# maxjiang93/space_time_pde

Hardware: AMD Instinct MI355X
Metric: query-points/sec (fwd+PDE-residual bwd), rb2d 128^3 latent (higher is better)
Workload: dtype f32; 1 GPU; BASELINE configs[1]: latent [1,32,128,128,32], 2^20 query points, RB2 (3 transport + continuity), ImNet nf=32 softplus, L1 losses, backward to ImNet + UNet3d parameters; points=1048576, parallelism=points sharded x1, unet=UNet3d(igres=(32, 128, 128), nf=16, mf=256) fwd+bwd inside the timed step

## Files before the change

### include/stpde_hip.h

```cpp
#ifndef STPDE_HIP_H
#define STPDE_HIP_H

#ifdef __cplusplus
extern "C" {
#endif

#define STPDE_OK 0
#define STPDE_E_BADARG 1
#define STPDE_E_UNSUPPORTED 2
#define STPDE_E_LAUNCH 3

#define STPDE_ACT_TANH 0
#define STPDE_ACT_RELU 1
#define STPDE_ACT_SOFTPLUS 2
#define STPDE_ACT_ELU 3
#define STPDE_ACT_SWISH 4
#define STPDE_ACT_LEAKYRELU 5

#define STPDE_XT 3
#define STPDE_PBAR_SLOTS 64

typedef struct {
  int S1;
  int S2;
  int pair0[6];
  int pair1[6];
  int act;
  float act_param;
  int combo;
  float alpha[6];
} stpde_jet_cfg;

int stpde_version(void);
int stpde_last_error(char* buf, unsigned long n);
#define STPDE_TUNE_CONV3_LDS_OFF 0
#define STPDE_TUNE_CONV3_LDS_MINBLK 1
#define STPDE_TUNE_CONV3_LDS_GX 2
#define STPDE_TUNE_CONV_WGRAD_LDS_GX 3
#define STPDE_TUNE_CONV1_WGRAD_LDS_GX 4
#define STPDE_TUNE_WGRAD_FP32_SWAP 5
#define STPDE_TUNE_FC2_BWD_FUSED 6
#define STPDE_TUNE_COUNT 7
int stpde_tune(const char* name, int value);
int stpde_trace_enable(int on);
long stpde_trace_read(char* buf, unsigned long n);

typedef struct {
  int P, N, B, n0, n1, n2, C;
  int p_base;
  float lo_c[3], hi_c[3], cube[3];
  float alpha[6];
} stpde_gather_desc;
int stpde_lig_gather(const stpde_gather_desc* d, const float* pts, const float* latent, float* X, float* XR,
                     float* coef, int* cell, float* cw , void* stream);

typedef struct {
  int ntiles, KT, MT, first_hidden;
  stpde_jet_cfg cfg;
  int mfma_bf16;
  int packed;
  int det;
} stpde_layer_desc;
int stpde_jet_layer_fwd(const stpde_layer_desc* d, const float* in_pre, const float* X, const float* Wh_pack,
                        const float* Ws_pack, const float* tanc, const float* W0s_pack, const float* tanc0,
                        float* out_pre, const float* cw ,
                        const void* Wh_pack_bf16, float* z0, void* stream);

int stpde_jet_tail_fwd(const stpde_jet_cfg* cfg, int ntiles, int nf16, const float* in_pre2, const float* X,
                       const float* const* Wh_pack, const float* const* Ws_pack, const float* const* tanc,
                       float* const* out_pre, const float* cw, void* stream);

int stpde_jet_tail_fwd_p(const stpde_jet_cfg* cfg, int ntiles, int nf16, const float* in_pre2, const float* X,
                         const float* const* Wh_pack, const float* const* Ws_pack, const float* const* tanc,
                         float* const* out_pre, const float* cw, int packed, const void* const* Wh16_pack, void* stream);

int stpde_jet_tail_bwd(const stpde_jet_cfg* cfg, int ntiles, int nf16, const float* abar5, const float* const* WhT_pack,
                       const float* const* pre, float* const* abar_out, const float* cw, float* act_param_bar,
                       void* stream);

int stpde_jet_tail_bwd_p(const stpde_jet_cfg* cfg, int ntiles, int nf16, const float* abar5, const float* const* WhT_pack,
                         const float* const* pre, float* const* abar_out, const float* cw, float* act_param_bar, int packed,
                         const void* const* WhT16_pack, void* stream);

int stpde_jet_layer_bwd(const stpde_layer_desc* d, const float* abar_out, const float* WhT_pack, float* in_pre,
                        const float* X, const float* W0s_pack, const float* tanc0, float* abar0, const float* cw,
                        float* act_param_bar, const void* WhT_pack_bf16 ,
                        float* abar0_tan, const float* z0, void* stream);

int stpde_jet_layer_bwd_to(const stpde_layer_desc* d, const float* abar_out, const float* WhT_pack, const float* in_pre,
                           float* abar_in, const float* cw, float* act_param_bar, const void* WhT_pack_bf16, void* stream);

int stpde_jet_wgrad(const stpde_layer_desc* d, int SP, const float* abar_out, const float* in_pre, const float* X,
                    const float* tanc0, float* dW_aug, const float* cw, void* stream);

int stpde_jet_fc1_bwd_supported(const stpde_layer_desc* d);
int stpde_jet_fc1_bwd(const stpde_layer_desc* d, const float* abar1, const void* WhT_pack_bf16, const float* z0,
                      const float* tanc0, const float* cw, const float* X, float* abar0, float* abar0_tan, float* dW_aug,
                      float* act_param_bar, void* stream);

int stpde_jet_fc2_bwd_supported(const stpde_layer_desc* d);
int stpde_jet_fc2_bwd(const stpde_layer_desc* d, const float* abar2, const float* WhT_pack, const float* pre1, const float* X,
                      const float* cw, float* abar1, float* dW_aug, float* act_param_bar, void* stream);

int stpde_lig_reduce_fwd(const stpde_jet_cfg* cfg, int S_mlp, int P, int n_out, const float* out_pre,
                         const float* coef, float* jets, long ldp, void* stream);
int stpde_lig_reduce_bwd(const stpde_jet_cfg* cfg, int S_mlp, int P, int n_out, const float* jets_bar, long ldp,
                         const float* coef, float* abar_out, void* stream);

int stpde_jet_tan0_reduce(int ntiles, int MT, const float* abar0_tan, float* dW_aug, int ldw, int det ,
                          void* stream);

typedef struct {
  int ntiles, nlayers, C, n1, n2;
  int MT[8];
  int SP[8];
  int packed[8];
  int S[8];
} stpde_xbar_desc;
int stpde_lig_xbar_scatter(const stpde_xbar_desc* d, const float* const* abar, const float* const* WsL_pack,
                           const int* cell, float* dlatent, void* stream);
int stpde_lig_xbar_rows(const stpde_xbar_desc* d, const float* const* abar, const float* const* WsL_pack,
                        float* xrows, void* stream);
int stpde_lig_dlatent_reduce(int B, int n0, int n1, int n2, int C, const float* xrows, const int* perm,
                             const int* start, float* dlatent, void* stream);

// ... 56 lines not shown
                        void* stream);

typedef struct {
  int P, N, B, dim, C;
  int n[4];
  float lo_c[4], hi_c[4], cube[4];
} stpde_interp_desc;
int stpde_interp_fwd(const stpde_interp_desc* d, const float* grid, const float* pts, float* out ,
                     float* corner_values , float* weights ,
                     float* x_relative , void* stream);
int stpde_interp_bwd_grid(const stpde_interp_desc* d, const float* pts, const float* out_bar,
                          const float* corner_bar, float* dgrid, void* stream);

typedef struct {
  int D, P, N, B, C;
  int p_base;
  int ntiles;
  int n[4];
  float lo_c[4], hi_c[4], cube[4];
} stpde_gather_nd_desc;
int stpde_lig_gather_nd(const stpde_gather_nd_desc* d, const float* pts, const float* latent, float* X,
                        float* cw , void* stream);
int stpde_lig_reduce_nd_fwd(int D, int P, int ntiles, int n_out, const float* out_pre ,
                            const float* cw, float* y, long ldp, void* stream);

int stpde_lig_reduce_nd_bwd(int D, int P, int ntiles, int n_out, const float* y_bar, long ldp, const float* cw,
                            float* abar_out , void* stream);
int stpde_lig_cell_nd(const stpde_gather_nd_desc* d, const float* pts, int* cell , void* stream);
int stpde_lig_dlatent_reduce_nd(int D, int B, const int* n , int C, const float* xrows, const int* perm,
                                const int* start, float* dlatent, void* stream);

int stpde_lig_coef_nd(const stpde_gather_nd_desc* d, const float* pts, float* coef , void* stream);
int stpde_lig_reduce_nd_jet_fwd(const stpde_jet_cfg* cfg, int S_mlp, int D, int P, int ntiles, int n_out,
                                const float* out_pre , const float* coef,
                                float* jets , long ldp, void* stream);

int stpde_lig_reduce_nd_jet_bwd(const stpde_jet_cfg* cfg, int S_mlp, int D, int P, int ntiles, int n_out,
                                const float* jets_bar , long ldp, const float* coef,
                                float* abar_out , void* stream);
int stpde_jet_wgrad_nd(const stpde_layer_desc* d, int SP, const float* abar_out, const float* in_pre, const float* X,
                       const float* tanc0, float* dW_aug, const float* cw, int ncoord, void* stream);
int stpde_jet_tan0_reduce_nd(int ntiles, int MT, const float* abar0_tan, float* dW_aug, int ldw, int det, int ncoord, void* stream);

typedef struct {
  int B, T, Z, X, Ci, Co, ksize;
  int det;
  int mfma_bf16;
} stpde_conv3d_desc;
#define STPDE_DET_K 6
int stpde_det_finalize(const void* acc, long n, float* out, void* stream);
int stpde_conv3d_fwd(const stpde_conv3d_desc* d, const float* x, const float* w_pack, const float* bias, float* y,
                     void* stream);
int stpde_conv3d_wgrad(const stpde_conv3d_desc* d, const float* x, const float* ybar, float* dW, void* stream);
int stpde_conv3d_wgrad_bias(const stpde_conv3d_desc* d, const float* x, const float* ybar, float* dW, float* dbias,
                            void* stream);

typedef struct {
  stpde_conv3d_desc d;
  const float* x;
  const float* w_pack;
  const float* bias;
  float* y;
  const float* x2;
  const float* w2_pack;
  float* y2;
  const float* wo2_pack;
  const float* bias2;
  const double* in_sums;
  const float* in_gamma;
  const float* in_beta;
  float* in_running_mean;
  float* in_running_var;
  float* in_stat;
  double* out_sums;
  const float* m;
  const float* m_stat;
  const float* m_gamma;
  const float* m_beta;
  float* m_bsum;
  int Ci2, Co2;
  float in_eps, in_momentum;
} stpde_conv3d_fused_args;
int stpde_conv3d_fused(const stpde_conv3d_fused_args* a, int* epilogue_done, void* stream);
int stpde_conv3d_wgrad_onload(const stpde_conv3d_desc* d, const float* x, const float* ybar, float* dW, float* dbias,
                              const float* in_stat, const float* in_gamma, const float* in_beta, void* stream);

#define STPDE_BN_REP 16
typedef struct {
  long N;
  int C, training, relu;
  float eps, momentum;
  int scratch_zeroed;
  int stats_mode;
  int reduce_done;
  int det;
} stpde_bn_desc;
int stpde_bn_fwd(const stpde_bn_desc* d, const float* x, const float* residual, const float* gamma, const float* beta,
                 float* running_mean, float* running_var, float* sums, float* stat, float* y, void* stream);
int stpde_bn_bwd(const stpde_bn_desc* d, const float* x, const float* y, const float* dy, const float* gamma,
                 const float* stat, float* bsum, float* dx, float* dresidual, float* dgamma, float* dbeta, void* stream);

typedef struct {
  int B, T, Z, X, C, ft, fz, fx;
} stpde_resample_desc;
int stpde_resample3d(const stpde_resample_desc* d, int mode, const float* in, const float* aux, float* out,
                     void* stream);

#define STPDE_RES_MAX_INS 192
enum {
  STPDE_RES_JET = 0, STPDE_RES_X, STPDE_RES_CONST, STPDE_RES_ADD, STPDE_RES_SUB, STPDE_RES_MUL, STPDE_RES_DIV,
  STPDE_RES_NEG, STPDE_RES_POWI, STPDE_RES_SIN, STPDE_RES_COS, STPDE_RES_EXP, STPDE_RES_LOG, STPDE_RES_SQRT,
  STPDE_RES_TANH, STPDE_RES_ABS, STPDE_RES_OUT,
  STPDE_RES_TAN, STPDE_RES_SINH, STPDE_RES_COSH, STPDE_RES_ASIN, STPDE_RES_ACOS, STPDE_RES_ATAN, STPDE_RES_ATAN2,
  STPDE_RES_POWC, STPDE_RES_POW, STPDE_RES_MIN, STPDE_RES_MAX, STPDE_RES_SIGN, STPDE_RES_STEP,
  STPDE_RES_LT, STPDE_RES_LE, STPDE_RES_EQ, STPDE_RES_NE, STPDE_RES_AND, STPDE_RES_OR, STPDE_RES_NOT,
  STPDE_RES_SEL, STPDE_RES_STEPC
};
#define STPDE_RES_SEL_THEN(b) ((int)((unsigned)(b) & 0xffffu))
#define STPDE_RES_SEL_ELSE(b) ((int)((unsigned)(b) >> 16))
typedef struct {
  int op, a, b;
  float c;
} stpde_res_ins;
int stpde_residual_fwd(const stpde_res_ins* prog_dev, int nins, int n_eq, int n_out, int P, const float* jets,
                       long ld_stream, long ld_channel, const float* x , float* res, void* stream);
int stpde_residual_bwd(const stpde_res_ins* prog_dev, int nins, int n_eq, int n_out, int P, const float* jets,
                       long ld_stream, long ld_channel, const float* x, const float* res_bar, float* jets_bar,
                       void* stream);
#define STPDE_RES_MAX_COEF 8
typedef struct {
  int n;
  int n_per_batch;
  int det;
  int per_batch[STPDE_RES_MAX_COEF];
  const float* value[STPDE_RES_MAX_COEF];
  float* bar[STPDE_RES_MAX_COEF];
} stpde_res_coefs;
int stpde_residual_coef_fwd(const stpde_res_ins* prog_dev, int nins, int n_eq, int n_out, int P, const float* jets,
                            long ld_stream, long ld_channel, const float* x, float* res, const stpde_res_coefs* coefs,
                            void* stream);
int stpde_residual_coef_bwd(const stpde_res_ins* prog_dev, int nins, int n_eq, int n_out, int P, const float* jets,
                            long ld_stream, long ld_channel, const float* x, const float* res_bar, float* jets_bar,
                            const stpde_res_coefs* coefs, void* stream);

#define STPDE_LOSS_L1 0
#define STPDE_LOSS_L2 1
#define STPDE_LOSS_HUBER 2
#define STPDE_LOSS_DET 16
int stpde_loss_sum(int kind, long n, const float* a, const float* b, float* out_sum, void* stream);
int stpde_loss_grad(int kind, long n, const float* a, const float* b, const float* grad_sum_dev, float* grad_a,
                    void* stream);

typedef struct {
  long n;
  float clip, beta1, beta2, eps, weight_decay, step_size, bias2_sqrt;
} stpde_adam_desc;
int stpde_clip_adam(const stpde_adam_desc* d, float* param, const float* grad, float* exp_avg, float* exp_avg_sq,
                    void* stream);
typedef struct {
  float* p;
  const float* g;
  float* m;
  float* v;
  long n;
  float step_size, bias2_sqrt;
} stpde_adam_tensor;
// ... 96 lines not shown
```

### space_time_pde_amd/_lib.py

```python
import ctypes as C
import os
import subprocess
import threading

_HERE = os.path.dirname(os.path.abspath(__file__))
_CSRC = os.path.join(_HERE, "csrc")
LIB_PATH = os.environ.get("STPDE_LIB") or os.path.join(_HERE, "libstpde_hip.so")
_SOURCES = ["jet_layer.hip", "jet_layer_s00.hip", "jet_layer_s03.hip", "jet_layer_s30.hip", "jet_layer_s31.hip", "jet_layer_s32.hip", "jet_layer_s34.hip", "jet_layer_s36.hip", "jet_tail.hip", "jet_wgrad.hip", "jet_wgrad_s00.hip", "jet_wgrad_s30.hip", "jet_wgrad_s31.hip", "jet_wgrad_s32.hip", "jet_wgrad_s34.hip", "jet_wgrad_s36.hip", "jet_fc1_bwd.hip", "jet_fc2_bwd.hip", "lig_gather_reduce.hip", "lig_pipeline.hip", "interp_nd.hip", "conv3d.hip", "conv3d_fused.hip", "optim.hip", "residual.hip", "bn.hip", "resample.hip", "sampler.hip", "sampler_median.hip", "api.cpp"]
_HIPFLAGS = ["--offload-arch=gfx950", "-O3", "-std=c++17", "-fPIC", "-ffp-contract=off", "-munsafe-fp-atomics",
             "--offload-compress"]

ABI_VERSION = 316

ACT_CODES = {"tanh": 0, "relu": 1, "softplus": 2, "elu": 3, "swish": 4, "leakyrelu": 5}
PBAR_SLOTS = 64
XT = 3


class JetCfg(C.Structure):
    _fields_ = [("S1", C.c_int), ("S2", C.c_int), ("pair0", C.c_int * 6), ("pair1", C.c_int * 6),
                ("act", C.c_int), ("act_param", C.c_float), ("combo", C.c_int), ("alpha", C.c_float * 6)]


class GatherDesc(C.Structure):
# ... 175 lines not shown
        objs.append(o)
        ostamp = o + ".srchash"
        owant = _source_hash([s] + _includes(s))
        if not force and os.path.exists(o) and os.path.exists(ostamp) and open(ostamp).read().strip() == owant:
            continue
        flags = _HIPFLAGS if s.endswith(".hip") else ["-O3", "-std=c++17", "-fPIC"]
        cmd = ["hipcc"] + flags + ["-c", s, "-o", o]
        if verbose:
            print(" ".join(cmd))
        procs.append((cmd, ostamp, owant, subprocess.Popen(cmd, stdout=subprocess.PIPE, stderr=subprocess.STDOUT)))
    for cmd, ostamp, owant, p in procs:
        out, _ = p.communicate()
        if p.returncode != 0:
            raise RuntimeError("hipcc failed: %s\n%s" % (" ".join(cmd), out.decode()))
        with open(ostamp, "w") as f:
            f.write(owant)
    cmd = ["hipcc", "--offload-arch=gfx950", "--offload-compress", "-shared", "-fPIC", "-o", LIB_PATH] + objs
    r = subprocess.run(cmd, stdout=subprocess.PIPE, stderr=subprocess.STDOUT)
    if r.returncode != 0:
        raise RuntimeError("link failed: %s\n%s" % (" ".join(cmd), r.stdout.decode()))
    with open(stamp, "w") as f:
        f.write(want)
    return LIB_PATH


_lib = None
_lock = threading.Lock()
_VP = C.c_void_p

_SIGNATURES = {
    "stpde_version": ([], C.c_int),
    "stpde_last_error": ([C.c_char_p, C.c_ulong], C.c_int),
    "stpde_tune": ([C.c_char_p, C.c_int], C.c_int),
    "stpde_trace_enable": ([C.c_int], C.c_int),
    "stpde_trace_read": ([C.c_char_p, C.c_ulong], C.c_long),
    "stpde_lig_gather": ([C.POINTER(GatherDesc), _VP, _VP, _VP, _VP, _VP, _VP, _VP, _VP], C.c_int),
    "stpde_lig_gather_nd": ([C.POINTER(GatherNdDesc), _VP, _VP, _VP, _VP, _VP], C.c_int),
    "stpde_lig_reduce_nd_fwd": ([C.c_int, C.c_int, C.c_int, C.c_int, _VP, _VP, _VP, C.c_long, _VP], C.c_int),
    "stpde_lig_reduce_nd_bwd": ([C.c_int, C.c_int, C.c_int, C.c_int, _VP, C.c_long, _VP, _VP, _VP], C.c_int),
    "stpde_lig_cell_nd": ([C.POINTER(GatherNdDesc), _VP, _VP, _VP], C.c_int),
    "stpde_lig_dlatent_reduce_nd": ([C.c_int, C.c_int, C.POINTER(C.c_int), C.c_int, _VP, _VP, _VP, _VP, _VP], C.c_int),
    "stpde_lig_coef_nd": ([C.POINTER(GatherNdDesc), _VP, _VP, _VP], C.c_int),
    "stpde_lig_reduce_nd_jet_fwd": ([C.POINTER(JetCfg), C.c_int, C.c_int, C.c_int, C.c_int, C.c_int, _VP, _VP, _VP, C.c_long,
                                     _VP], C.c_int),
    "stpde_lig_reduce_nd_jet_bwd": ([C.POINTER(JetCfg), C.c_int, C.c_int, C.c_int, C.c_int, C.c_int, _VP, C.c_long, _VP, _VP,
                                     _VP], C.c_int),
    "stpde_jet_wgrad_nd": ([C.POINTER(LayerDesc), C.c_int] + [_VP] * 6 + [C.c_int, _VP], C.c_int),
    "stpde_jet_tan0_reduce_nd": ([C.c_int, C.c_int, _VP, _VP, C.c_int, C.c_int, C.c_int, _VP], C.c_int),
    "stpde_jet_layer_fwd": ([C.POINTER(LayerDesc)] + [_VP] * 12, C.c_int),
    "stpde_jet_layer_bwd": ([C.POINTER(LayerDesc)] + [_VP] * 13, C.c_int),
    "stpde_jet_layer_bwd_to": ([C.POINTER(LayerDesc)] + [_VP] * 8, C.c_int),
    "stpde_jet_tail_fwd": ([C.POINTER(JetCfg), C.c_int, C.c_int, _VP, _VP, C.POINTER(_VP), C.POINTER(_VP), C.POINTER(_VP),
                            C.POINTER(_VP), _VP, _VP], C.c_int),
    "stpde_jet_tail_bwd": ([C.POINTER(JetCfg), C.c_int, C.c_int, _VP, C.POINTER(_VP), C.POINTER(_VP), C.POINTER(_VP), _VP,
                            _VP, _VP], C.c_int),
    "stpde_jet_tail_fwd_p": ([C.POINTER(JetCfg), C.c_int, C.c_int, _VP, _VP, C.POINTER(_VP), C.POINTER(_VP), C.POINTER(_VP),
                              C.POINTER(_VP), _VP, C.c_int, C.POINTER(_VP), _VP], C.c_int),
    "stpde_jet_tail_bwd_p": ([C.POINTER(JetCfg), C.c_int, C.c_int, _VP, C.POINTER(_VP), C.POINTER(_VP), C.POINTER(_VP), _VP,
                              _VP, C.c_int, C.POINTER(_VP), _VP], C.c_int),
    "stpde_jet_tan0_reduce": ([C.c_int, C.c_int, _VP, _VP, C.c_int, C.c_int, _VP], C.c_int),
    "stpde_jet_wgrad": ([C.POINTER(LayerDesc), C.c_int] + [_VP] * 7, C.c_int),
    "stpde_jet_fc1_bwd_supported": ([C.POINTER(LayerDesc)], C.c_int),
    "stpde_jet_fc1_bwd": ([C.POINTER(LayerDesc)] + [_VP] * 11, C.c_int),
    "stpde_jet_fc2_bwd_supported": ([C.POINTER(LayerDesc)], C.c_int),
    "stpde_jet_fc2_bwd": ([C.POINTER(LayerDesc)] + [_VP] * 9, C.c_int),
    "stpde_lig_reduce_fwd": ([C.POINTER(JetCfg), C.c_int, C.c_int, C.c_int, _VP, _VP, _VP, C.c_long, _VP], C.c_int),
    "stpde_lig_reduce_bwd": ([C.POINTER(JetCfg), C.c_int, C.c_int, C.c_int, _VP, C.c_long, _VP, _VP, _VP], C.c_int),
    "stpde_lig_xbar_scatter": ([C.POINTER(XbarDesc), C.POINTER(_VP), C.POINTER(_VP), _VP, _VP, _VP], C.c_int),
    "stpde_lig_xbar_rows": ([C.POINTER(XbarDesc), C.POINTER(_VP), C.POINTER(_VP), _VP, _VP], C.c_int),
    "stpde_lig_dlatent_reduce": ([C.c_int] * 5 + [_VP] * 5, C.c_int),
    "stpde_lig_imnet_jet_fwd": ([C.POINTER(ImNetPlanDesc), C.POINTER(JetCfg), C.POINTER(JetCfg), C.POINTER(GatherDesc), _VP,
                                 _VP, C.POINTER(LigWorkspace), _VP, C.c_long, C.c_int, _VP], C.c_int),
    "stpde_lig_imnet_jet_bwd": ([C.POINTER(ImNetPlanDesc), C.POINTER(JetCfg), C.POINTER(JetCfg), C.POINTER(JetCfg),
                                 C.POINTER(GatherDesc), C.POINTER(LigWorkspace), _VP, C.c_long, _VP, _VP, _VP, C.c_int, _VP],
                                C.c_int),
    "stpde_lig_sort_tmp_bytes": ([C.c_int, C.c_long], C.c_ulong),
    "stpde_lig_cell_sort": ([C.c_int, C.c_long, _VP, _VP, _VP, _VP, C.c_ulong, _VP], C.c_int),
    "stpde_interp_fwd": ([C.POINTER(InterpDesc)] + [_VP] * 7, C.c_int),
    "stpde_interp_bwd_grid": ([C.POINTER(InterpDesc)] + [_VP] * 5, C.c_int),
    "stpde_conv3d_fwd": ([C.POINTER(Conv3dDesc)] + [_VP] * 5, C.c_int),
    "stpde_conv3d_wgrad": ([C.POINTER(Conv3dDesc)] + [_VP] * 4, C.c_int),
    "stpde_conv3d_wgrad_bias": ([C.POINTER(Conv3dDesc)] + [_VP] * 5, C.c_int),
    "stpde_conv3d_fused": ([C.POINTER(Conv3dFusedArgs), C.POINTER(C.c_int), _VP], C.c_int),
    "stpde_conv3d_wgrad_onload": ([C.POINTER(Conv3dDesc)] + [_VP] * 8, C.c_int),
    "stpde_residual_fwd": ([_VP, C.c_int, C.c_int, C.c_int, C.c_int, _VP, C.c_long, C.c_long, _VP, _VP, _VP], C.c_int),
    "stpde_residual_bwd": ([_VP, C.c_int, C.c_int, C.c_int, C.c_int, _VP, C.c_long, C.c_long, _VP, _VP, _VP, _VP],
                           C.c_int),
    "stpde_residual_coef_fwd": ([_VP, C.c_int, C.c_int, C.c_int, C.c_int, _VP, C.c_long, C.c_long, _VP, _VP,
                                 C.POINTER(ResCoefs), _VP], C.c_int),
    "stpde_residual_coef_bwd": ([_VP, C.c_int, C.c_int, C.c_int, C.c_int, _VP, C.c_long, C.c_long, _VP, _VP, _VP,
                                 C.POINTER(ResCoefs), _VP], C.c_int),
    "stpde_resample3d": ([C.POINTER(ResampleDesc), C.c_int, _VP, _VP, _VP, _VP], C.c_int),
    "stpde_det_finalize": ([_VP, C.c_long, _VP, _VP], C.c_int),
    "stpde_bn_fwd": ([C.POINTER(BnDesc)] + [_VP] * 10, C.c_int),
    "stpde_bn_bwd": ([C.POINTER(BnDesc)] + [_VP] * 11, C.c_int),
    "stpde_loss_sum": ([C.c_int, C.c_long, _VP, _VP, _VP, _VP], C.c_int),
    "stpde_loss_grad": ([C.c_int, C.c_long, _VP, _VP, _VP, _VP, _VP], C.c_int),
    "stpde_clip_adam": ([C.POINTER(AdamDesc)] + [_VP] * 5, C.c_int),
    "stpde_clip_adam_multi": ([C.POINTER(AdamDesc), _VP, _VP, C.c_int, C.c_int, _VP], C.c_int),
    "stpde_opt_advance": ([C.POINTER(OptDesc), _VP, _VP], C.c_int),
    "stpde_clip_adam_dev": ([C.POINTER(AdamDesc)] + [_VP] * 6, C.c_int),
    "stpde_clip_adam_multi_dev": ([C.POINTER(AdamDesc), _VP, _VP, _VP, C.c_int, C.c_int, _VP], C.c_int),
    "stpde_clip_sgd": ([C.POINTER(SgdDesc)] + [_VP] * 5, C.c_int),
    "stpde_clip_sgd_multi": ([C.POINTER(SgdDesc), _VP, _VP, _VP, C.c_int, C.c_int, _VP], C.c_int),
    "stpde_sampler_draw": ([C.POINTER(SamplerDesc)] + [_VP] * 4, C.c_int),
    "stpde_sampler_produce": ([C.POINTER(SamplerDesc)] + [_VP] * 10, C.c_int),
    "stpde_sampler_filter": ([C.POINTER(SamplerFilterDesc)] + [_VP] * 9, C.c_int),
    "stpde_sampler_produce_filtered": ([C.POINTER(SamplerDesc)] + [_VP] * 8, C.c_int),
    "stpde_sampler_median": ([C.POINTER(SamplerFilterDesc)] + [_VP] * 5, C.c_int),
}


def exported_symbols():
    return sorted(_SIGNATURES)


def register_signatures(sigs):
    _SIGNATURES.update(sigs)


def lib():
    global _lib
    if _lib is None:
        with _lock:
            if _lib is None:
                if not os.path.exists(LIB_PATH):
                    raise RuntimeError(
                        "libstpde_hip.so is not built (%s). Run `python -c 'import __graft_entry__ as g; g.build()'` "
                        "-- this package has no CPU/eager fallback for its HIP operators." % LIB_PATH)
                import torch
                h = C.CDLL(LIB_PATH)
                for name, (argtypes, restype) in _SIGNATURES.items():
                    fn = getattr(h, name)
                    fn.argtypes = argtypes
                    fn.restype = restype
                if h.stpde_version() != ABI_VERSION:
                    raise RuntimeError("libstpde_hip.so at %s has ABI version %d, this package needs %d: rebuild it "
                                       "(python -c 'import __graft_entry__ as g; g.build()')"
                                       % (LIB_PATH, h.stpde_version(), ABI_VERSION))
                _lib = h
    return _lib


_EXC = {1: ValueError, 2: NotImplementedError, 3: RuntimeError}


def check(rc):
    if rc != 0:
        buf = C.create_string_buffer(512)
        lib().stpde_last_error(buf, 512)
        raise _EXC.get(rc, RuntimeError)("libstpde_hip: " + buf.value.decode())


def tune(name, value):
    prev = lib().stpde_tune(name.encode(), int(value))
    if prev < 0:
        raise KeyError(name)
    _tune_values[name] = int(value)
    return prev


_tune_values = {}


def tune_value(name):
    return _tune_values.get(name, 0)
# ... 84 lines not shown
```

### space_time_pde_amd/csrc/api.cpp

```cpp
#include <hip/hip_runtime.h>

#include <cstdarg>
#include <cstdio>
#include <cstring>
#include <mutex>
#include <set>
#include <string>

#include "../../include/stpde_hip.h"

static thread_local char g_err[512] = "";

void stpde_set_error(const char* fmt, ...) {
  va_list ap;
  va_start(ap, fmt);
  vsnprintf(g_err, sizeof(g_err), fmt, ap);
  va_end(ap);
}

int stpde_check_launch(const char* what) {
  hipError_t e = hipGetLastError();
  if (e != hipSuccess) {
    stpde_set_error("%s: launch failed: %s", what, hipGetErrorString(e));
    return STPDE_E_LAUNCH;
  }
  return STPDE_OK;
}

extern "C" int stpde_version(void) { return 316; }

#include <atomic>
static const char* const g_tune_names[STPDE_TUNE_COUNT] = {"conv3_lds_off", "conv3_lds_minblk", "conv3_lds_gx", "conv_wgrad_lds_gx",
                                                           "conv1_wgrad_lds_gx", "wgrad_fp32_swap", "fc2_bwd_fused"};
static std::atomic<int> g_tune[STPDE_TUNE_COUNT];
int stpde_tune_get(int key) { return (key >= 0 && key < STPDE_TUNE_COUNT) ? g_tune[key].load(std::memory_order_relaxed) : 0; }
extern "C" int stpde_tune(const char* name, int value) {
  if (!name) return -1;
  for (int k = 0; k < STPDE_TUNE_COUNT; ++k)
    if (!strcmp(name, g_tune_names[k])) return g_tune[k].exchange(value);
  stpde_set_error("stpde_tune: unknown key '%s'", name);
  return -1;
}

extern "C" int stpde_last_error(char* buf, unsigned long n) {
  if (!buf || n == 0) return STPDE_E_BADARG;
  strncpy(buf, g_err, n - 1);
  buf[n - 1] = 0;
  return STPDE_OK;
}

int stpde_trace_on = 0;
static std::mutex g_trace_mu;
static std::set<std::string> g_trace;

void stpde_trace_note(const char* launcher, const char* kernel) {
  std::lock_guard<std::mutex> lk(g_trace_mu);
  g_trace.insert(std::string(kernel) + " @ " + launcher);
}

extern "C" int stpde_trace_enable(int on) {
  std::lock_guard<std::mutex> lk(g_trace_mu);
  g_trace.clear();
  stpde_trace_on = on ? 1 : 0;
  return STPDE_OK;
}

extern "C" long stpde_trace_read(char* buf, unsigned long n) {
  std::lock_guard<std::mutex> lk(g_trace_mu);
  std::string all;
  for (const auto& s : g_trace) all += s + "\n";
  if (buf && n > 0) {
    strncpy(buf, all.c_str(), n - 1);
    buf[n - 1] = 0;
  }
  return (long)all.size() + 1;
}
```

### space_time_pde_amd/csrc/conv3d_fused.hip

```cpp
#include <type_traits>
#include "common.h"
#include "conv_common.h"

struct FusedArgs {
  stpde_conv3d_fused_args f;
  int nvox;
};

template <int MC, int VT, bool K3, int DUAL, bool ONLOAD, int EPI, bool BF = false>
__global__ __launch_bounds__(256) void k_conv_fused(FusedArgs a) {
  static_assert(!(K3 && (DUAL || ONLOAD)), "dual / on-load variants are 1x1x1 only");
  static_assert(!BF || K3, "bf16 operands: 3x3x3 only");
  __shared__ float tab[ONLOAD ? 3 * 512 : 1];
  __shared__ double red[EPI ? 4 * MC * 16 * 2 : 1];
  const stpde_conv3d_desc& d = a.f.d;
  const int lane = threadIdx.x & 63;
  const int wv = threadIdx.x >> 6;
  const int g = lane >> 4, j = lane & 15;
  const int lo = lane * 4;
  const int Ci = d.Ci, Co = d.Co, KT = Ci / 16, MT1 = Co / 16;
  const int Co2 = DUAL == 1 ? a.f.Co2 : 0, MT2 = Co2 / 16, MT = MT1 + MT2;
  const int KT2 = DUAL == 2 ? a.f.Ci2 / 16 : 0;
  const int ntap = K3 ? 27 : 1;
  const long N = a.nvox;
  if (ONLOAD) {
    for (int c = threadIdx.x; c < Ci; c += 256) {
      float mean, var, rstd;
      bn_stat_f64(a.f.in_sums, Ci, c, N, a.f.in_eps, a.f.d.det, mean, var, rstd);
      const float gm = a.f.in_gamma ? a.f.in_gamma[c] : 1.f, bt = a.f.in_beta ? a.f.in_beta[c] : 0.f;
      tab[c] = mean;
      tab[512 + c] = rstd * gm;
      tab[1024 + c] = bt;
      if (blockIdx.x == 0 && blockIdx.y == 0) {
        a.f.in_stat[c] = mean;
        a.f.in_stat[Ci + c] = rstd;
        if (a.f.in_running_mean) {
          const float unb = N > 1 ? var * ((float)N / (float)(N - 1)) : var;
          a.f.in_running_mean[c] = (1.f - a.f.in_momentum) * a.f.in_running_mean[c] + a.f.in_momentum * mean;
          a.f.in_running_var[c] = (1.f - a.f.in_momentum) * a.f.in_running_var[c] + a.f.in_momentum * unb;
        }
      }
    }
    __syncthreads();
  }
  const int tile0 = (blockIdx.x * 4 + wv) * VT;
  const bool active = tile0 * 16 < a.nvox;
  int v[VT];
  bool vin[VT];
  VoxN vn[VT];
#pragma unroll
  for (int t = 0; t < VT; ++t) {
    v[t] = (tile0 + t) * 16 + j;
    vin[t] = v[t] < a.nvox;
    vn[t] = vox_prepare(d, vox_coords(d, vin[t] ? v[t] : 0));
    if (!vin[t]) vn[t].ok = 0u;
  }
  const int nvalid = active ? (a.nvox - tile0 * 16 < VT * 16 ? a.nvox - tile0 * 16 : VT * 16) : 0;
  for (int mt0 = blockIdx.y * MC; mt0 < MT; mt0 += gridDim.y * MC) {
    f32x4 acc[VT][MC];
#pragma unroll
    for (int t = 0; t < VT; ++t)
#pragma unroll
      for (int mi = 0; mi < MC; ++mi) acc[t][mi] = f32x4{0.f, 0.f, 0.f, 0.f};
    const float* wbase[MC];
    int wstride[MC];
#pragma unroll
    for (int mi = 0; mi < MC; ++mi) {
      const int mt = mt0 + mi < MT ? mt0 + mi : mt0;
      if (DUAL == 1 && mt >= MT1) {
        wbase[mi] = a.f.wo2_pack + (size_t)(mt - MT1) * 256 + lo;
        wstride[mi] = MT2 * 256;
      } else {
        wbase[mi] = a.f.w_pack + (size_t)mt * 256 + lo;
        wstride[mi] = MT1 * 256;
      }
    }
    if (active) {
      for (int tap = 0; tap < ntap; ++tap) {
        int nb[VT];
        const float* src[VT];
        unsigned tmask;
        int toff;
        tap_uniform(d, tap, tmask, toff);
#pragma unroll
        for (int t = 0; t < VT; ++t) {
          nb[t] = vin[t] ? tap_nb(vn[t], tmask, toff) : -1;
          src[t] = a.f.x + (size_t)(nb[t] < 0 ? 0 : nb[t]) * Ci + 4 * g;
        }
        for (int kt = 0; kt < KT; ++kt) {
          f32x4 B[VT];
          f32x4 mn, sc, bt;
          if (ONLOAD) {
            mn = *reinterpret_cast<const f32x4*>(tab + 16 * kt + 4 * g);
            sc = *reinterpret_cast<const f32x4*>(tab + 512 + 16 * kt + 4 * g);
            bt = *reinterpret_cast<const f32x4*>(tab + 1024 + 16 * kt + 4 * g);
          }
#pragma unroll
          for (int t = 0; t < VT; ++t) {
            B[t] = ld4(src[t] + 16 * kt);
            if (ONLOAD) {
              B[t] = (B[t] - mn) * sc + bt;
#pragma unroll
              for (int r = 0; r < 4; ++r) B[t][r] = B[t][r] > 0.f ? B[t][r] : 0.f;
            }
            if (nb[t] < 0) B[t] = f32x4{0.f, 0.f, 0.f, 0.f};
          }
          if constexpr (BF) {
            f32x4 w[MC];
#pragma unroll
            for (int mi = 0; mi < MC; ++mi) w[mi] = ld4(wbase[mi] + (size_t)(tap * KT + kt) * wstride[mi]);
            __builtin_amdgcn_sched_barrier(0);
            bf16x4 Bb[VT];
#pragma unroll
            for (int t = 0; t < VT; ++t) Bb[t] = cvt_bf4(B[t]);
#pragma unroll
            for (int mi = 0; mi < MC; ++mi) {
              const bf16x4 wb = cvt_bf4(w[mi]);
#pragma unroll
              for (int t = 0; t < VT; ++t) acc[t][mi] = mfma_bf16k(wb, Bb[t], acc[t][mi]);
            }
          } else {
#pragma unroll
            for (int mi = 0; mi < MC; ++mi) {
              const f32x4 w = ld4(wbase[mi] + (size_t)(tap * KT + kt) * wstride[mi]);
#pragma unroll
              for (int r = 0; r < 4; ++r)
#pragma unroll
                for (int t = 0; t < VT; ++t) acc[t][mi] = mfma4(w[r], B[t][r], acc[t][mi]);
            }
          }
        }
      }
      if (DUAL == 2) {
        const int C2 = a.f.Ci2;
        for (int kt = 0; kt < KT2; ++kt) {
          f32x4 B[VT];
#pragma unroll
          for (int t = 0; t < VT; ++t) {
            B[t] = ld4(a.f.x2 + (size_t)(vin[t] ? v[t] : 0) * C2 + 4 * g + 16 * kt);
            if (!vin[t]) B[t] = f32x4{0.f, 0.f, 0.f, 0.f};
          }
#pragma unroll
          for (int mi = 0; mi < MC; ++mi) {
            const int mt = mt0 + mi < MT ? mt0 + mi : mt0;
            const f32x4 w = ld4(a.f.w2_pack + ((size_t)kt * MT1 + mt) * 256 + lo);
#pragma unroll
            for (int r = 0; r < 4; ++r)
#pragma unroll
              for (int t = 0; t < VT; ++t) acc[t][mi] = mfma4(w[r], B[t][r], acc[t][mi]);
          }
        }
      }
    }
#pragma unroll
    for (int mi = 0; mi < MC; ++mi) {
      const int mt = mt0 + mi;
      const bool live = mt < MT;
      const bool second = DUAL == 1 && mt >= MT1;
      float* ybase = second ? a.f.y2 : a.f.y;
      const int ystride = second ? Co2 : Co;
// ... 299 lines not shown
          if (!(h[rr] > 0.f)) o[rr] = 0.f;
        s1 += o;
        s2 += o * xm * mrstd;
      }
      buf_st16(yr, vo[t], 0, o);
    }
    if constexpr (EPI != 0) {
      if (++nacc == FLUSH) flush();
    }
  }
  if constexpr (EPI != 0) {
    if (nacc) flush();
  }
  if constexpr (EPI != 0) {
    if (j == 15) {
#pragma unroll
      for (int rr = 0; rr < 4; ++rr) {
        red[(wv * 16 + 4 * g + rr) * 2] = sd1[rr];
        red[(wv * 16 + 4 * g + rr) * 2 + 1] = sd2[rr];
      }
    }
    __syncthreads();
    if (threadIdx.x < KT * 16) {
      const int m = threadIdx.x >> 4, c = threadIdx.x & 15;
      double t1 = 0., t2 = 0.;
      for (int w = m; w < 4; w += KT) {
        t1 += red[(w * 16 + c) * 2];
        t2 += red[(w * 16 + c) * 2 + 1];
      }
      const int rep = blockIdx.x % STPDE_BN_REP;
      if (a.f.d.det) {
        long long* acc = reinterpret_cast<long long*>(EPI == 1 ? (void*)a.f.out_sums : (void*)a.f.m_bsum);
        if (EPI == 1) {
          det_add_f64(acc + (size_t)(16 * m + c) * STPDE_DET_K, t1);
          det_add_f64(acc + ((size_t)C + 16 * m + c) * STPDE_DET_K, t2);
        } else {
          det_add_f32(acc + (size_t)(16 * m + c) * STPDE_DET_K, (float)t1);
          det_add_f32(acc + ((size_t)C + 16 * m + c) * STPDE_DET_K, (float)t2);
        }
      } else if (EPI == 1) {
        atomicAdd(a.f.out_sums + (size_t)(2 * rep) * C + 16 * m + c, t1);
        atomicAdd(a.f.out_sums + (size_t)(2 * rep + 1) * C + 16 * m + c, t2);
      } else {
        atomicAdd(a.f.m_bsum + (size_t)(2 * rep) * C + 16 * m + c, (float)t1);
        atomicAdd(a.f.m_bsum + (size_t)(2 * rep + 1) * C + 16 * m + c, (float)t2);
      }
    }
  }
}

template <int EPI>
static bool launch_conv3_lds(const FusedArgs& a0, hipStream_t st) {
  const stpde_conv3d_desc& d = a0.f.d;
  if (stpde_tune_get(STPDE_TUNE_CONV3_LDS_OFF) || d.ksize != 3 || d.Ci != d.Co || (d.Ci != 16 && d.Ci != 32 && d.Ci != 64)) return false;
  const int KT = d.Ci / 16;
  const int TZ = KT == 1 ? 4 : 2, TX = KT == 4 ? 16 : 32;
  if (d.T % 2 || d.Z % TZ || d.X % TX) return false;
  if ((size_t)d.B * d.T * d.Z * d.X * d.Ci * 4 >= (1u << 31)) return false;
  const int nblk = d.B * (d.T / 2) * (d.Z / TZ) * (d.X / TX);
  const int minblk_t = stpde_tune_get(STPDE_TUNE_CONV3_LDS_MINBLK);
  if (nblk < (minblk_t > 0 ? minblk_t : 1024)) return false;
  const int gx_env = stpde_tune_get(STPDE_TUNE_CONV3_LDS_GX);
  int gx = gx_env > 0 ? gx_env : 512;
  if (gx > nblk) gx = nblk;
  const FusedArgs& a = a0;
  const bool bf = d.mfma_bf16 == 1;
#define STPDE_C3L(K)                                                                  \
  if (KT == K && !bf) {                                                              \
    if constexpr (EPI == 0) STPDE_LAUNCH((k_conv3_lds<K, 0>), dim3(gx), dim3(256), 0, st, a); \
    if constexpr (EPI == 1) STPDE_LAUNCH((k_conv3_lds<K, 1>), dim3(gx), dim3(256), 0, st, a); \
    if constexpr (EPI == 2) STPDE_LAUNCH((k_conv3_lds<K, 2>), dim3(gx), dim3(256), 0, st, a); \
  }                                                                                  \
  if (KT == K && bf) {                                                               \
    if constexpr (EPI == 0) STPDE_LAUNCH((k_conv3_lds<K, 0, true>), dim3(gx), dim3(256), 0, st, a); \
    if constexpr (EPI == 1) STPDE_LAUNCH((k_conv3_lds<K, 1, true>), dim3(gx), dim3(256), 0, st, a); \
    if constexpr (EPI == 2) STPDE_LAUNCH((k_conv3_lds<K, 2, true>), dim3(gx), dim3(256), 0, st, a); \
  }
  STPDE_C3L(1) STPDE_C3L(2) STPDE_C3L(4)
#undef STPDE_C3L
  return true;
}

template <bool K3, int DUAL, bool ONLOAD, int EPI>
static void launch_fused(const FusedArgs& a, int MT, bool big, dim3 grid, hipStream_t st) {
  if constexpr (K3) {
    if (a.f.d.mfma_bf16 == 1) {
      if (big) {
        if (MT == 1)
          STPDE_LAUNCH((k_conv_fused<1, 4, K3, DUAL, ONLOAD, EPI, true>), grid, dim3(256), 0, st, a);
        else if (MT == 2)
          STPDE_LAUNCH((k_conv_fused<2, 4, K3, DUAL, ONLOAD, EPI, true>), grid, dim3(256), 0, st, a);
        else
          STPDE_LAUNCH((k_conv_fused<4, 4, K3, DUAL, ONLOAD, EPI, true>), grid, dim3(256), 0, st, a);
      } else {
        if (MT == 1)
          STPDE_LAUNCH((k_conv_fused<1, 1, K3, DUAL, ONLOAD, EPI, true>), grid, dim3(256), 0, st, a);
        else if (MT == 2)
          STPDE_LAUNCH((k_conv_fused<2, 1, K3, DUAL, ONLOAD, EPI, true>), grid, dim3(256), 0, st, a);
        else
          STPDE_LAUNCH((k_conv_fused<4, 1, K3, DUAL, ONLOAD, EPI, true>), grid, dim3(256), 0, st, a);
      }
      return;
    }
  }
  if (big) {
    if (MT == 1)
      STPDE_LAUNCH((k_conv_fused<1, 4, K3, DUAL, ONLOAD, EPI>), grid, dim3(256), 0, st, a);
    else if (MT == 2)
      STPDE_LAUNCH((k_conv_fused<2, 4, K3, DUAL, ONLOAD, EPI>), grid, dim3(256), 0, st, a);
    else
      STPDE_LAUNCH((k_conv_fused<4, 4, K3, DUAL, ONLOAD, EPI>), grid, dim3(256), 0, st, a);
  } else {
    if (MT == 1)
      STPDE_LAUNCH((k_conv_fused<1, 1, K3, DUAL, ONLOAD, EPI>), grid, dim3(256), 0, st, a);
    else if (MT == 2)
      STPDE_LAUNCH((k_conv_fused<2, 1, K3, DUAL, ONLOAD, EPI>), grid, dim3(256), 0, st, a);
    else
      STPDE_LAUNCH((k_conv_fused<4, 1, K3, DUAL, ONLOAD, EPI>), grid, dim3(256), 0, st, a);
  }
}

extern "C" int stpde_conv3d_fused(const stpde_conv3d_fused_args* f, int* epilogue_done, void* stream) {
  if (!f) {
    stpde_set_error("conv3d_fused: null arguments");
    return STPDE_E_BADARG;
  }
  const stpde_conv3d_desc* d = &f->d;
  if (d->B < 1 || d->T < 1 || d->Z < 1 || d->X < 1 || d->Ci < 16 || d->Co < 16 || (d->Ci & 15) || (d->Co & 15) ||
      (d->ksize != 1 && d->ksize != 3) || (size_t)d->B * d->T * d->Z * d->X >= (1u << 31) / 16) {
    stpde_set_error("conv3d_fused: bad descriptor (channels must be multiples of 16, ksize 1 or 3)");
    return STPDE_E_BADARG;
  }
  const bool dual_out = f->y2 != nullptr, dual_in = f->x2 != nullptr, onload = f->in_sums != nullptr;
  const bool stats = f->out_sums != nullptr, mask = f->m != nullptr;
  if (stpde_check_conv_mode(d, "conv3d_fused")) return STPDE_E_BADARG;
  if (!f->x || !f->w_pack || !f->y || (dual_out && (!f->wo2_pack || f->Co2 < 16 || (f->Co2 & 15))) ||
      (dual_in && (!f->w2_pack || f->Ci2 < 16 || (f->Ci2 & 15))) || (onload && (!f->in_stat || d->Ci > 512)) ||
      (mask && (!f->m_stat || !f->m_bsum)) || (d->ksize == 3 && (dual_out || dual_in || onload)) ||
      (dual_out + dual_in + onload + mask > 1) || (stats && (dual_in || mask))) {
    stpde_set_error("conv3d_fused: inconsistent arguments");
    return STPDE_E_BADARG;
  }
  if (epilogue_done) *epilogue_done = 1;
  FusedArgs a{};
  a.f = *f;
  a.nvox = d->B * d->T * d->Z * d->X;
  const hipStream_t st = (hipStream_t)stream;
  const int ntiles = (a.nvox + 15) / 16;
  const int MT = d->Co / 16 + (dual_out ? f->Co2 / 16 : 0);
  const int nchunks = (MT + 3) / 4;
  const bool big = ntiles >= 16384;
  dim3 grid;
  if (big) {
    grid = dim3((ntiles + 15) / 16, 1);
  } else {
    const int gx = (ntiles + 3) / 4;
    const int gy = gx >= 1024 ? 1 : nchunks;
    if (d->ksize == 3 && gx * gy < 256 && !d->det) {
      int rc = stpde_conv3d_fwd(d, f->x, f->w_pack, f->bias, f->y, stream);
      if (rc) return rc;
      if (stats) rc = stpde_bn_stats_f64(f->y, a.nvox, d->Co, f->out_sums, st);
      if (mask && epilogue_done) *epilogue_done = 0;
      if (mask && !epilogue_done) {
        stpde_set_error("conv3d_fused: tap-split volume needs epilogue_done");
        return STPDE_E_BADARG;
      }
      return rc;
    }
    grid = dim3(gx, gy);
  }
  if (d->ksize == 3) {
    if (stats ? launch_conv3_lds<1>(a, st) : (mask ? launch_conv3_lds<2>(a, st) : launch_conv3_lds<0>(a, st)))
      return stpde_check_launch("k_conv3_lds");
    if (stats)
      launch_fused<true, 0, false, 1>(a, MT, big, grid, st);
    else if (mask)
      launch_fused<true, 0, false, 2>(a, MT, big, grid, st);
    else
      launch_fused<true, 0, false, 0>(a, MT, big, grid, st);
  } else if (dual_out) {
    if (stats)
      launch_fused<false, 1, false, 1>(a, MT, big, grid, st);
    else
      launch_fused<false, 1, false, 0>(a, MT, big, grid, st);
  } else if (dual_in) {
    launch_fused<false, 2, false, 0>(a, MT, big, grid, st);
  } else if (onload) {
    if (stats)
      launch_fused<false, 0, true, 1>(a, MT, big, grid, st);
    else
      launch_fused<false, 0, true, 0>(a, MT, big, grid, st);
  } else if (mask) {
    launch_fused<false, 0, false, 2>(a, MT, big, grid, st);
  } else if (stats) {
    launch_fused<false, 0, false, 1>(a, MT, big, grid, st);
  } else {
    launch_fused<false, 0, false, 0>(a, MT, big, grid, st);
  }
  return stpde_check_launch("k_conv_fused");
}
```

Measured before the change: 2.559 million query-points/s.

## Add software-pipelined operand loads for small fused conv volumes

Adds a PIPE variant of the fused conv kernel that keeps a 16-deep register ring of prefetched activation and weight vectors, so global load latency overlaps with MFMA work on small, latency-bound volumes. A new plan function picks this path when the grid would be under 256 blocks and tap-splitting does not apply. For those cases it splits output tiles one per block (MC=1, gy=MT) to add parallelism. The tradeoff is higher register pressure and possibly lower occupancy; a tune knob can turn the path off.

```diff
diff --git a/include/stpde_hip.h b/include/stpde_hip.h
--- a/include/stpde_hip.h
+++ b/include/stpde_hip.h
@@ -40,7 +40,8 @@
 #define STPDE_TUNE_CONV1_WGRAD_LDS_GX 4
 #define STPDE_TUNE_WGRAD_FP32_SWAP 5
 #define STPDE_TUNE_FC2_BWD_FUSED 6
-#define STPDE_TUNE_COUNT 7
+#define STPDE_TUNE_CONV_SMALL_PIPE 7
+#define STPDE_TUNE_COUNT 8
 int stpde_tune(const char* name, int value);
 int stpde_trace_enable(int on);
 long stpde_trace_read(char* buf, unsigned long n);
@@ -263,6 +264,10 @@
   float in_eps, in_momentum;
 } stpde_conv3d_fused_args;
 int stpde_conv3d_fused(const stpde_conv3d_fused_args* a, int* epilogue_done, void* stream);
+#define STPDE_CONV_PLAN_PLAIN 0
+#define STPDE_CONV_PLAN_PIPE 1
+#define STPDE_CONV_PLAN_TAPSPLIT 2
+int stpde_conv3d_fused_plan(int nvox, int MT, int ksize, int det, int* MC, int* VT, int* gx, int* gy);
 int stpde_conv3d_wgrad_onload(const stpde_conv3d_desc* d, const float* x, const float* ybar, float* dW, float* dbias,
                               const float* in_stat, const float* in_gamma, const float* in_beta, void* stream);
 
diff --git a/space_time_pde_amd/_lib.py b/space_time_pde_amd/_lib.py
--- a/space_time_pde_amd/_lib.py
+++ b/space_time_pde_amd/_lib.py
@@ -281,6 +281,7 @@
     "stpde_conv3d_wgrad": ([C.POINTER(Conv3dDesc)] + [_VP] * 4, C.c_int),
     "stpde_conv3d_wgrad_bias": ([C.POINTER(Conv3dDesc)] + [_VP] * 5, C.c_int),
     "stpde_conv3d_fused": ([C.POINTER(Conv3dFusedArgs), C.POINTER(C.c_int), _VP], C.c_int),
+    "stpde_conv3d_fused_plan": ([C.c_int] * 4 + [C.POINTER(C.c_int)] * 4, C.c_int),
     "stpde_conv3d_wgrad_onload": ([C.POINTER(Conv3dDesc)] + [_VP] * 8, C.c_int),
     "stpde_residual_fwd": ([_VP, C.c_int, C.c_int, C.c_int, C.c_int, _VP, C.c_long, C.c_long, _VP, _VP, _VP], C.c_int),
     "stpde_residual_bwd": ([_VP, C.c_int, C.c_int, C.c_int, C.c_int, _VP, C.c_long, C.c_long, _VP, _VP, _VP, _VP],
diff --git a/space_time_pde_amd/csrc/api.cpp b/space_time_pde_amd/csrc/api.cpp
--- a/space_time_pde_amd/csrc/api.cpp
+++ b/space_time_pde_amd/csrc/api.cpp
@@ -31,7 +31,7 @@
 
 #include <atomic>
 static const char* const g_tune_names[STPDE_TUNE_COUNT] = {"conv3_lds_off", "conv3_lds_minblk", "conv3_lds_gx", "conv_wgrad_lds_gx",
-                                                           "conv1_wgrad_lds_gx", "wgrad_fp32_swap", "fc2_bwd_fused"};
+                                                           "conv1_wgrad_lds_gx", "wgrad_fp32_swap", "fc2_bwd_fused", "conv_small_pipe"};
 static std::atomic<int> g_tune[STPDE_TUNE_COUNT];
 int stpde_tune_get(int key) { return (key >= 0 && key < STPDE_TUNE_COUNT) ? g_tune[key].load(std::memory_order_relaxed) : 0; }
 extern "C" int stpde_tune(const char* name, int value) {
diff --git a/space_time_pde_amd/csrc/conv3d_fused.hip b/space_time_pde_amd/csrc/conv3d_fused.hip
--- a/space_time_pde_amd/csrc/conv3d_fused.hip
+++ b/space_time_pde_amd/csrc/conv3d_fused.hip
@@ -7,10 +7,13 @@
   int nvox;
 };
 
-template <int MC, int VT, bool K3, int DUAL, bool ONLOAD, int EPI, bool BF = false>
+constexpr int PIPE_D = 16;
+
+template <int MC, int VT, bool K3, int DUAL, bool ONLOAD, int EPI, bool BF = false, bool PIPE = false>
 __global__ __launch_bounds__(256) void k_conv_fused(FusedArgs a) {
   static_assert(!(K3 && (DUAL || ONLOAD)), "dual / on-load variants are 1x1x1 only");
   static_assert(!BF || K3, "bf16 operands: 3x3x3 only");
+  static_assert(!PIPE || (MC == 1 && VT == 1), "pipelined operand loads: one output tile, one voxel tile per wave");
   __shared__ float tab[ONLOAD ? 3 * 512 : 1];
   __shared__ double red[EPI ? 4 * MC * 16 * 2 : 1];
   const stpde_conv3d_desc& d = a.f.d;
@@ -75,7 +78,72 @@
         wstride[mi] = MT1 * 256;
       }
     }
-    if (active) {
+    if constexpr (PIPE) {
+      if (active) {
+        const int S1 = ntap * KT, S = S1 + KT2;
+        const float* x2p = nullptr;
+        const float* w2p = nullptr;
+        if (DUAL == 2) {
+          x2p = a.f.x2 + (size_t)(vin[0] ? v[0] : 0) * a.f.Ci2 + 4 * g;
+          w2p = a.f.w2_pack + (size_t)mt0 * 256 + lo;
+        }
+        int ps = 0, ptap = 0, pkt = 0;
+        const float* pb;
+        bool pneg;
+        auto settap = [&](int tap) {
+          unsigned tmask;
+          int toff;
+          tap_uniform(d, tap, tmask, toff);
+          const int nb = vin[0] ? tap_nb(vn[0], tmask, toff) : -1;
+          pb = a.f.x + (size_t)(nb < 0 ? 0 : nb) * Ci + 4 * g;
+          pneg = nb < 0;
+        };
+        settap(0);
+        auto fetch = [&](f32x4& Bs, f32x4& Ws, bool& Zs) {
+          const bool sec = DUAL == 2 && ps >= S1;
+          Bs = ld4(sec ? x2p + 16 * (ps - S1) : pb + 16 * pkt);
+          Ws = ld4(sec ? w2p + (size_t)(ps - S1) * MT1 * 256 : wbase[0] + (size_t)ps * wstride[0]);
+          Zs = sec ? !vin[0] : pneg;
+          if (ps + 1 < S) {
+            ++ps;
+            if (ps < S1 && ++pkt == KT) {
+              pkt = 0;
+              settap(++ptap);
+            }
+          }
+        };
+        f32x4 pB[PIPE_D], pW[PIPE_D];
+        bool pZ[PIPE_D];
+#pragma unroll
+        for (int i = 0; i < PIPE_D - 1; ++i) fetch(pB[i], pW[i], pZ[i]);
+        for (int s0 = 0; s0 < S; s0 += PIPE_D) {
+#pragma unroll
+          for (int i = 0; i < PIPE_D; ++i) {
+            fetch(pB[(i + PIPE_D - 1) % PIPE_D], pW[(i + PIPE_D - 1) % PIPE_D], pZ[(i + PIPE_D - 1) % PIPE_D]);
+            const int s = s0 + i;
+            if (s < S) {
+              f32x4 B = pB[i];
+              if (ONLOAD) {
+                const f32x4 mn = *reinterpret_cast<const f32x4*>(tab + 16 * s + 4 * g);
+                const f32x4 sc = *reinterpret_cast<const f32x4*>(tab + 512 + 16 * s + 4 * g);
+                const f32x4 bt = *reinterpret_cast<const f32x4*>(tab + 1024 + 16 * s + 4 * g);
+                B = (B - mn) * sc + bt;
+#pragma unroll
+                for (int r = 0; r < 4; ++r) B[r] = B[r] > 0.f ? B[r] : 0.f;
+              }
+              if (pZ[i]) B = f32x4{0.f, 0.f, 0.f, 0.f};
+              const f32x4 w = pW[i];
+              if constexpr (BF) {
+                acc[0][0] = mfma_bf16k(cvt_bf4(w), cvt_bf4(B), acc[0][0]);
+              } else {
+#pragma unroll
+                for (int r = 0; r < 4; ++r) acc[0][0] = mfma4(w[r], B[r], acc[0][0]);
+              }
+            }
+          }
+        }
+      }
+    } else if (active) {
       for (int tap = 0; tap < ntap; ++tap) {
         int nb[VT];
         const float* src[VT];
@@ -541,20 +609,22 @@
 }
 
 template <bool K3, int DUAL, bool ONLOAD, int EPI>
-static void launch_fused(const FusedArgs& a, int MT, bool big, dim3 grid, hipStream_t st) {
+static void launch_fused(const FusedArgs& a, int MC, bool big, bool pipe, dim3 grid, hipStream_t st) {
   if constexpr (K3) {
     if (a.f.d.mfma_bf16 == 1) {
-      if (big) {
-        if (MT == 1)
+      if (pipe) {
+        STPDE_LAUNCH((k_conv_fused<1, 1, K3, DUAL, ONLOAD, EPI, true, true>), grid, dim3(256), 0, st, a);
+      } else if (big) {
+        if (MC == 1)
           STPDE_LAUNCH((k_conv_fused<1, 4, K3, DUAL, ONLOAD, EPI, true>), grid, dim3(256), 0, st, a);
-        else if (MT == 2)
+        else if (MC == 2)
           STPDE_LAUNCH((k_conv_fused<2, 4, K3, DUAL, ONLOAD, EPI, true>), grid, dim3(256), 0, st, a);
         else
           STPDE_LAUNCH((k_conv_fused<4, 4, K3, DUAL, ONLOAD, EPI, true>), grid, dim3(256), 0, st, a);
       } else {
-        if (MT == 1)
+        if (MC == 1)
           STPDE_LAUNCH((k_conv_fused<1, 1, K3, DUAL, ONLOAD, EPI, true>), grid, dim3(256), 0, st, a);
-        else if (MT == 2)
+        else if (MC == 2)
           STPDE_LAUNCH((k_conv_fused<2, 1, K3, DUAL, ONLOAD, EPI, true>), grid, dim3(256), 0, st, a);
         else
           STPDE_LAUNCH((k_conv_fused<4, 1, K3, DUAL, ONLOAD, EPI, true>), grid, dim3(256), 0, st, a);
@@ -562,21 +632,47 @@
       return;
     }
   }
-  if (big) {
-    if (MT == 1)
+  if (pipe) {
+    STPDE_LAUNCH((k_conv_fused<1, 1, K3, DUAL, ONLOAD, EPI, false, true>), grid, dim3(256), 0, st, a);
+  } else if (big) {
+    if (MC == 1)
       STPDE_LAUNCH((k_conv_fused<1, 4, K3, DUAL, ONLOAD, EPI>), grid, dim3(256), 0, st, a);
-    else if (MT == 2)
+    else if (MC == 2)
       STPDE_LAUNCH((k_conv_fused<2, 4, K3, DUAL, ONLOAD, EPI>), grid, dim3(256), 0, st, a);
     else
       STPDE_LAUNCH((k_conv_fused<4, 4, K3, DUAL, ONLOAD, EPI>), grid, dim3(256), 0, st, a);
   } else {
-    if (MT == 1)
+    if (MC == 1)
       STPDE_LAUNCH((k_conv_fused<1, 1, K3, DUAL, ONLOAD, EPI>), grid, dim3(256), 0, st, a);
-    else if (MT == 2)
+    else if (MC == 2)
       STPDE_LAUNCH((k_conv_fused<2, 1, K3, DUAL, ONLOAD, EPI>), grid, dim3(256), 0, st, a);
     else
       STPDE_LAUNCH((k_conv_fused<4, 1, K3, DUAL, ONLOAD, EPI>), grid, dim3(256), 0, st, a);
   }
+}
+
+extern "C" int stpde_conv3d_fused_plan(int nvox, int MT, int ksize, int det, int* MC, int* VT, int* gx, int* gy) {
+  if (nvox < 1 || MT < 1 || (ksize != 1 && ksize != 3) || !MC || !VT || !gx || !gy) {
+    stpde_set_error("conv3d_fused_plan: bad argument");
+    return -1;
+  }
+  const int ntiles = (nvox + 15) / 16;
+  *MC = MT == 1 ? 1 : (MT == 2 ? 2 : 4);
+  if (ntiles >= 16384) {
+    *VT = 4;
+    *gx = (ntiles + 15) / 16;
+    *gy = 1;
+    return STPDE_CONV_PLAN_PLAIN;
+  }
+  *VT = 1;
+  *gx = (ntiles + 3) / 4;
+  *gy = *gx >= 1024 ? 1 : (MT + 3) / 4;
+  if (*gx * *gy >= 256) return STPDE_CONV_PLAN_PLAIN;
+  if (ksize == 3 && !det) return STPDE_CONV_PLAN_TAPSPLIT;
+  if (stpde_tune_get(STPDE_TUNE_CONV_SMALL_PIPE) == 2) return STPDE_CONV_PLAN_PLAIN;
+  *MC = 1;
+  *gy = MT;
+  return STPDE_CONV_PLAN_PIPE;
 }
 
 extern "C" int stpde_conv3d_fused(const stpde_conv3d_fused_args* f, int* epilogue_done, void* stream) {
@@ -605,56 +701,49 @@
   a.f = *f;
   a.nvox = d->B * d->T * d->Z * d->X;
   const hipStream_t st = (hipStream_t)stream;
-  const int ntiles = (a.nvox + 15) / 16;
   const int MT = d->Co / 16 + (dual_out ? f->Co2 / 16 : 0);
-  const int nchunks = (MT + 3) / 4;
-  const bool big = ntiles >= 16384;
-  dim3 grid;
-  if (big) {
-    grid = dim3((ntiles + 15) / 16, 1);
-  } else {
-    const int gx = (ntiles + 3) / 4;
-    const int gy = gx >= 1024 ? 1 : nchunks;
-    if (d->ksize == 3 && gx * gy < 256 && !d->det) {
-      int rc = stpde_conv3d_fwd(d, f->x, f->w_pack, f->bias, f->y, stream);
-      if (rc) return rc;
-      if (stats) rc = stpde_bn_stats_f64(f->y, a.nvox, d->Co, f->out_sums, st);
-      if (mask && epilogue_done) *epilogue_done = 0;
-      if (mask && !epilogue_done) {
-        stpde_set_error("conv3d_fused: tap-split volume needs epilogue_done");
-        return STPDE_E_BADARG;
-      }
-      return rc;
-    }
-    grid = dim3(gx, gy);
+  int MC, VT, gx, gy;
+  const int plan = stpde_conv3d_fused_plan(a.nvox, MT, d->ksize, d->det, &MC, &VT, &gx, &gy);
+  const bool big = VT == 4, pipe = plan == STPDE_CONV_PLAN_PIPE;
+  const dim3 grid(gx, gy);
+  if (plan == STPDE_CONV_PLAN_TAPSPLIT) {
+    int rc = stpde_conv3d_fwd(d, f->x, f->w_pack, f->bias, f->y, stream);
+    if (rc) return rc;
+    if (stats) rc = stpde_bn_stats_f64(f->y, a.nvox, d->Co, f->out_sums, st);
+    if (mask && epilogue_done) *epilogue_done = 0;
+    if (mask && !epilogue_done) {
+      stpde_set_error("conv3d_fused: tap-split volume needs epilogue_done");
+      return STPDE_E_BADARG;
+    }
+    return rc;
   }
   if (d->ksize == 3) {
     if (stats ? launch_conv3_lds<1>(a, st) : (mask ? launch_conv3_lds<2>(a, st) : launch_conv3_lds<0>(a, st)))
       return stpde_check_launch("k_conv3_lds");
     if (stats)
-      launch_fused<true, 0, false, 1>(a, MT, big, grid, st);
+      launch_fused<true, 0, false, 1>(a, MC, big, pipe, grid, st);
     else if (mask)
-      launch_fused<true, 0, false, 2>(a, MT, big, grid, st);
+      launch_fused<true, 0, false, 2>(a, MC, big, pipe, grid, st);
     else
-      launch_fused<true, 0, false, 0>(a, MT, big, grid, st);
+      launch_fused<true, 0, false, 0>(a, MC, big, pipe, grid, st);
   } else if (dual_out) {
     if (stats)
-      launch_fused<false, 1, false, 1>(a, MT, big, grid, st);
+      launch_fused<false, 1, false, 1>(a, MC, big, pipe, grid, st);
     else
-      launch_fused<false, 1, false, 0>(a, MT, big, grid, st);
+      launch_fused<false, 1, false, 0>(a, MC, big, pipe, grid, st);
   } else if (dual_in) {
-    launch_fused<false, 2, false, 0>(a, MT, big, grid, st);
+    launch_fused<false, 2, false, 0>(a, MC, big, pipe, grid, st);
   } else if (onload) {
     if (stats)
-      launch_fused<false, 0, true, 1>(a, MT, big, grid, st);
+      launch_fused<false, 0, true, 1>(a, MC, big, pipe, grid, st);
     else
-      launch_fused<false, 0, true, 0>(a, MT, big, grid, st);
+      launch_fused<false, 0, true, 0>(a, MC, big, pipe, grid, st);
   } else if (mask) {
-    launch_fused<false, 0, false, 2>(a, MT, big, grid, st);
+    launch_fused<false, 0, false, 2>(a, MC, big, pipe, grid, st);
   } else if (stats) {
-    launch_fused<false, 0, false, 1>(a, MT, big, grid, st);
+    launch_fused<false, 0, false, 1>(a, MC, big, pipe, grid, st);
   } else {
-    launch_fused<false, 0, false, 0>(a, MT, big, grid, st);
+    launch_fused<false, 0, false, 0>(a, MC, big, pipe, grid, st);
   }
   return stpde_check_launch("k_conv_fused");
 }
```

After: 2.581 million query-points/s, median of 6. Within noise of the previous version (+0.9%).
